# fu5ha/rayn

Hardware: NVIDIA H100
Metric: Msamples/sec (pixels x spp) (higher is better)
Workload: dtype f32

## Files before the change

### rayn_b200/csrc/api.cu

```cuda
#include <cuda_runtime.h>
#include <dlfcn.h>
#include <limits.h>
#include <stdarg.h>
#include <stdio.h>
#include <string.h>

#include <algorithm>
#include <array>
#include <string>
#include <vector>

#include "rt_accum.cuh"
#include "rt_denoise.cuh"
#include "rt_first_hit.cuh"
#include "rt_kernels.cuh"
#include "rt_temporal.cuh"
#ifdef RAYN_LEGACY_KERNELS
#include "rt_legacy.cuh"
#endif

using namespace rt;

static thread_local std::string g_last_error;

// ... 27 lines not shown
  float* d_slabs = nullptr;
  size_t cap_slabs = 0;
};

struct PassBuf {
  void** ptr;
  size_t per_path, per_slot, per_tile, fixed;
};
static const int N_PASS_BUFS = 23;

struct JobPlane {
  float* user;
  int floats;
};

struct RaynContext {
  int device = 0;
  int flags = 0;
  cudaStream_t stream = nullptr;
  std::string err;
  bool has_scene = false;
  DevScene scene;
  int64_t cap_paths = 0;
  size_t pass_cap[N_PASS_BUFS] = {};
  PassBufs pb;
  int* d_tile_ids = nullptr;
  int* d_batch_prefix = nullptr;
  int* d_work_ctr = nullptr;
  int n_sm = 148;
  int occ_ext[2][SDFV_COUNT], occ_shd[SDFV_COUNT], occ_nrm[SDFV_COUNT], occ_nrm_trap[SDFV_COUNT];
  int occ_pre = 8, occ_post = 8, occ_sph = 8;
  int occ_pre_trap = 8, occ_post_trap = 8;
  int sdf_var[RAYN_MAX_HITABLES];
  struct Div3Check { float min_r2, fixed_r2; bool ok; };
  std::vector<Div3Check> div3_cache;
  float *d_s1 = nullptr, *d_s2 = nullptr, *d_scr = nullptr, *d_fis = nullptr;
  size_t cap_s1 = 0, cap_s2 = 0, cap_scr = 0;
  float* d_planes = nullptr;
  size_t cap_planes = 0;
  int* d_pack_ids = nullptr;
  size_t cap_pack_ids = 0;
  unsigned char* d_post = nullptr;
  size_t cap_post = 0;
// ... 47 lines not shown
    if (r_ != 0)                                                                                     \
      return fail(ctx, RAYN_ERR_NCCL, "%s: %s (%s:%d)", #call, g_nccl.GetErrorString ? g_nccl.GetErrorString(r_) : "?", __FILE__, __LINE__); \
  } while (0)

template <class T>
static cudaError_t regrow(T** p, size_t* cap, size_t need) {
  if (need <= *cap && *p) return cudaSuccess;
  if (*p) cudaFree(*p);
  *p = nullptr;
  *cap = 0;
  cudaError_t e = cudaMalloc((void**)p, std::max<size_t>(need, 1) * sizeof(T));
  if (e == cudaSuccess) *cap = need;
  return e;
}

static std::array<PassBuf, N_PASS_BUFS> pass_table(RaynContext* c, int QS, int seg_per_path, int lc_ns, bool trap) {
  PassBufs& p = c->pb;
  const size_t nseg = (QS + SEG_SLOTS - 1) / SEG_SLOTS;
  return {{
      {(void**)&p.o_time, sizeof(float4), 0, 0, 0},
      {(void**)&p.d_t, sizeof(float4), 0, 0, 0},
      {(void**)&p.rad, sizeof(float4), 0, 0, 0},
      {(void**)&p.thr, sizeof(float4), 0, 0, 0},
      {(void**)&p.nrm0, sizeof(float4), 0, 0, 0},
      {(void**)&p.term, sizeof(uint32_t), 0, 0, 0},
      {(void**)&p.q_live, sizeof(int), 0, 0, 0},
      {(void**)&p.q_key, sizeof(int), 0, 0, 0},
      {(void**)&p.q_shade, 0, sizeof(int), 0, 0},
      {(void**)&p.n_live, 0, 0, sizeof(int), 0},
      {(void**)&p.n_slots, 0, 0, sizeof(int), 0},
      {(void**)&p.bin_start, 0, 0, (RAYN_MAX_HITABLES + 1) * sizeof(int), 0},
      {(void**)&c->d_tile_ids, 0, 0, sizeof(int), 0},
      {(void**)&c->d_batch_prefix, 0, 0, sizeof(int), sizeof(int)},
      {(void**)&p.seg_cnt, 0, 0, nseg * RAYN_MAX_HITABLES * sizeof(int), 0},
      {(void**)&p.slot_prefix, 0, 0, (1 + RAYN_MAX_HITABLES) * sizeof(int), (1 + RAYN_MAX_HITABLES) * sizeof(int)},
      {(void**)&p.nrm, sizeof(float4), 0, 0, 0},
      {(void**)&p.vis, sizeof(uint32_t), 0, 0, 0},
      {(void**)&p.seg_a, (size_t)seg_per_path * sizeof(float4), 0, 0, 0},
      {(void**)&p.seg_b, (size_t)seg_per_path * sizeof(float4), 0, 0, 0},
      {(void**)&p.lc_c, (size_t)lc_ns * sizeof(float4), 0, 0, 0},
      {(void**)&p.lc_t, lc_ns > 4 ? 8 * sizeof(float) : 0, 0, 0, 0},
      {(void**)&p.trap_s, trap ? sizeof(float) : 0, 0, 0, 0},
  }};
}

static void free_pass(RaynContext* c) {
  for (const PassBuf& b : pass_table(c, 0, 0, 0, false)) {
    cudaFree(*b.ptr);
    *b.ptr = nullptr;
  }
  unsigned long long* counters = c->pb.counters;
  memset(&c->pb, 0, sizeof c->pb);
  c->pb.counters = counters;
  memset(c->pass_cap, 0, sizeof c->pass_cap);
}

static size_t pass_bytes_per_path(RaynContext* c, int R, int QS, int seg_per_path, int lc_ns, bool trap) {
  size_t bytes = 0;
  for (const PassBuf& b : pass_table(c, QS, seg_per_path, lc_ns, trap))
    bytes += b.per_path + (b.per_slot ? (size_t)(((double)QS / R) * b.per_slot + 1) : 0);
  return bytes;
}

static int32_t ensure_pass(RaynContext* ctx, int n_tiles, int R, int QS, int seg_per_path, int n_sdf, int lc_ns, bool trap) {
  const int64_t need_paths = (int64_t)n_tiles * R, need_q = (int64_t)n_tiles * QS;
  const std::array<PassBuf, N_PASS_BUFS> table = pass_table(ctx, QS, seg_per_path, lc_ns, trap);
  size_t need[N_PASS_BUFS];
  bool fits = true;
  for (int i = 0; i < N_PASS_BUFS; ++i) {
    const PassBuf& b = table[i];
    need[i] = b.per_path * need_paths + b.per_slot * need_q + b.per_tile * n_tiles + b.fixed;
    fits = fits && need[i] <= ctx->pass_cap[i];
  }
  if (fits) return RAYN_OK;
  free_pass(ctx);
  for (int i = 0; i < N_PASS_BUFS; ++i) {
    if (need[i] == 0) continue;
    const cudaError_t e = cudaMalloc(table[i].ptr, need[i]);
    if (e != cudaSuccess) {
      cudaGetLastError();
      free_pass(ctx);
      return fail(ctx, e == cudaErrorMemoryAllocation ? RAYN_ERR_OOM : RAYN_ERR_CUDA, "pass buffers (%lld paths): %s", (long long)need_paths,
                  cudaGetErrorString(e));
    }
    ctx->pass_cap[i] = need[i];
  }
  ctx->pb.prefix_stride = n_tiles + 1;
  ctx->pb.seg_cap = n_sdf > 0 ? need_paths * seg_per_path / n_sdf : 0;
  return RAYN_OK;
}

static void timed_begin(RaynContext* ctx, int kernel) {
  if (!(ctx->flags & RAYN_FLAG_TIMING)) return;
  if (ctx->timed_used == ctx->timed.size()) {
    TimedLaunch t;
    t.kernel = kernel;
    cudaEventCreate(&t.a);
    cudaEventCreate(&t.b);
    ctx->timed.push_back(t);
  }
  ctx->timed[ctx->timed_used].kernel = kernel;
  cudaEventRecord(ctx->timed[ctx->timed_used].a, ctx->stream);
}
// ... 67 lines not shown
  if (cudaGetDeviceCount(&ndev) != cudaSuccess || ndev == 0) {
    cudaGetLastError();
    return fail(nullptr, RAYN_ERR_NO_DEVICE, "no CUDA device: the rayn_b200 render path has no CPU fallback");
  }
  const int dev = cfg ? cfg->device : 0;
  if (dev < 0 || dev >= ndev) return fail(nullptr, RAYN_ERR_INVALID_ARG, "device %d out of range (have %d)", dev, ndev);
#ifndef RAYN_LEGACY_KERNELS
  if (cfg && (cfg->flags & RAYN_FLAG_SIMPLE_MARCH))
    return fail(nullptr, RAYN_ERR_UNSUPPORTED, "RAYN_FLAG_SIMPLE_MARCH needs the test build (librayn_b200_legacy.so, -DRAYN_LEGACY_KERNELS)");
#endif
  CU(cudaSetDevice(dev));
  ctx = new RaynContext();
  ctx->device = dev;
  ctx->flags = cfg ? cfg->flags : 0;
  ctx->cap_paths = (cfg && cfg->max_paths_per_pass > 0) ? cfg->max_paths_per_pass : (int64_t)96 << 20;
  memset(&ctx->pb, 0, sizeof ctx->pb);
  memset(&ctx->stats, 0, sizeof ctx->stats);
  memset(&ctx->scene, 0, sizeof ctx->scene);
  cudaError_t e = cudaStreamCreateWithFlags(&ctx->stream, cudaStreamNonBlocking);
  if (e == cudaSuccess) e = cudaMalloc(&ctx->pb.counters, CNT_TOTAL * sizeof(unsigned long long));
  if (e == cudaSuccess) e = cudaMalloc(&ctx->d_fis, RAYN_FIS_TABLE_SIZE * sizeof(float));
  if (e == cudaSuccess) e = cudaMalloc(&ctx->d_work_ctr, WC_TOTAL * sizeof(int));
  if (e == cudaSuccess) e = cudaMalloc(&ctx->d_kat, sizeof(unsigned long long));
  if (e == cudaSuccess) e = cudaDeviceGetAttribute(&ctx->n_sm, cudaDevAttrMultiProcessorCount, dev);
  if (e == cudaSuccess) e = cudaEventCreate(&ctx->ev0);
  if (e == cudaSuccess) e = cudaEventCreate(&ctx->ev1);
  for (int v = 0; v < SDFV_COUNT && e == cudaSuccess; ++v) {
    DISPATCH_SDFV(v, e = cudaOccupancyMaxActiveBlocksPerMultiprocessor(&ctx->occ_ext[0][v], k_extend_march<V, false>, EXT_T, 0);
                  if (e == cudaSuccess) e = cudaOccupancyMaxActiveBlocksPerMultiprocessor(&ctx->occ_ext[1][v], k_extend_march<V, true>, EXT_T, 0);
                  if (e == cudaSuccess) e = cudaOccupancyMaxActiveBlocksPerMultiprocessor(&ctx->occ_shd[v], k_shadow<V>, SHD_T, 0);
                  if (e == cudaSuccess) e = cudaOccupancyMaxActiveBlocksPerMultiprocessor(&ctx->occ_nrm[v], k_normals<V, false>, SLOT_BLOCK, 0);
                  if (e == cudaSuccess) e = cudaOccupancyMaxActiveBlocksPerMultiprocessor(&ctx->occ_nrm_trap[v], k_normals<V, true>, SLOT_BLOCK, 0));
  }
  if (e == cudaSuccess) e = cudaOccupancyMaxActiveBlocksPerMultiprocessor(&ctx->occ_pre, k_shade_pre<false>, SLOT_BLOCK, 0);
  if (e == cudaSuccess) e = cudaOccupancyMaxActiveBlocksPerMultiprocessor(&ctx->occ_post, k_shade_post<false>, SLOT_BLOCK, 0);
  if (e == cudaSuccess) e = cudaOccupancyMaxActiveBlocksPerMultiprocessor(&ctx->occ_pre_trap, k_shade_pre<true>, SLOT_BLOCK, 0);
  if (e == cudaSuccess) e = cudaOccupancyMaxActiveBlocksPerMultiprocessor(&ctx->occ_post_trap, k_shade_post<true>, SLOT_BLOCK, 0);
  if (e == cudaSuccess) e = cudaOccupancyMaxActiveBlocksPerMultiprocessor(&ctx->occ_sph, k_extend_spheres, EXT_BATCH, 0);
  if (e != cudaSuccess) {
    cudaGetLastError();
    fail(nullptr, RAYN_ERR_CUDA, "context setup: %s", cudaGetErrorString(e));
    if (ctx->stream) cudaStreamDestroy(ctx->stream);
    cudaFree(ctx->pb.counters), cudaFree(ctx->d_fis), cudaFree(ctx->d_work_ctr), cudaFree(ctx->d_kat);
    if (ctx->ev0) cudaEventDestroy(ctx->ev0);
    if (ctx->ev1) cudaEventDestroy(ctx->ev1);
    delete ctx;
    return RAYN_ERR_CUDA;
  }
  *out_ctx = ctx;
  return RAYN_OK;
}

int32_t rayn_b200_comm_destroy(RaynContext* ctx) {
  if (!ctx) return RAYN_ERR_INVALID_ARG;
  RaynComm& c = ctx->comm;
  cudaSetDevice(ctx->device);
  cudaStreamSynchronize(ctx->stream);
  if (c.comm && g_nccl.CommDestroy) g_nccl.CommDestroy(c.comm);
  cudaFree(c.d_table), cudaFree(c.d_slabs);
  c = RaynComm();
  return RAYN_OK;
}

void rayn_b200_destroy(RaynContext* ctx) {
  if (!ctx) return;
  cudaSetDevice(ctx->device);
  cudaStreamSynchronize(ctx->stream);
  rayn_b200_comm_destroy(ctx);
  free_pass(ctx);
  cudaFree(ctx->pb.counters);
  cudaFree(ctx->d_work_ctr);
  cudaFree(ctx->d_kat);
  cudaFree(ctx->d_pack_ids);
  cudaFree(ctx->d_post);
  cudaFree(ctx->d_s1), cudaFree(ctx->d_s2), cudaFree(ctx->d_scr), cudaFree(ctx->d_fis), cudaFree(ctx->d_planes);
  cudaFree(ctx->d_prev);
  for (auto& t : ctx->timed) cudaEventDestroy(t.a), cudaEventDestroy(t.b);
  if (ctx->graph_exec) cudaGraphExecDestroy(ctx->graph_exec);
  cudaEventDestroy(ctx->ev0), cudaEventDestroy(ctx->ev1);
  cudaStreamDestroy(ctx->stream);
  delete ctx;
}

static int32_t validate_scene(RaynContext* ctx, const RaynSceneDesc* s) {
  if (!s) return fail(ctx, RAYN_ERR_INVALID_ARG, "scene is NULL");
  if (s->n_hitables < 1 || s->n_hitables > RAYN_MAX_HITABLES)
    return fail(ctx, RAYN_ERR_INVALID_ARG, "n_hitables %d not in [1,%d]", s->n_hitables, RAYN_MAX_HITABLES);
  if (s->n_materials < 1 || s->n_materials > RAYN_MAX_MATERIALS)
    return fail(ctx, RAYN_ERR_INVALID_ARG, "n_materials %d not in [1,%d]", s->n_materials, RAYN_MAX_MATERIALS);
  if (s->n_lights < 0 || s->n_lights > RAYN_MAX_LIGHTS)
    return fail(ctx, RAYN_ERR_INVALID_ARG, "n_lights %d not in [0,%d]", s->n_lights, RAYN_MAX_LIGHTS);
  if (!s->hitables || !s->materials || (s->n_lights && !s->lights)) return fail(ctx, RAYN_ERR_INVALID_ARG, "NULL scene array");
  for (int i = 0; i < s->n_hitables; ++i) {
    const RaynHitable& h = s->hitables[i];
    if (h.kind < 0 || h.kind > RAYN_HITABLE_MANDELBULB) return fail(ctx, RAYN_ERR_INVALID_ARG, "hitable %d: bad kind %d", i, h.kind);
// ... 123 lines not shown
}

}

struct FramePlan {
  DevFrame fr;
  int R, QS, np, wpc;
  bool simple, traps, fold_all, volume_on;
  int fold_pre, n_fold, ns, seg_per_path, lc_ns;
};

struct Job {
  FramePlan P;
  PassBufs pb;
  int tiles_per_pass;
};

static unsigned resident(const RaynContext* ctx, const Job& J, int occ) {
  const int64_t max_blocks = (int64_t)J.pb.n_tiles * ((J.P.QS + SLOT_BLOCK - 1) / SLOT_BLOCK);
  return (unsigned)std::max<int64_t>(1, std::min<int64_t>((int64_t)ctx->n_sm * occ, max_blocks));
}

static int32_t frame_check(RaynContext* ctx, const RaynFrameDesc* f, bool tiles_given, FramePlan* P) {
  if (f->width <= 0 || f->height <= 0 || f->tile_w <= 0 || f->tile_h <= 0 || f->samples <= 0 || f->max_bounces < 0)
    return fail(ctx, RAYN_ERR_INVALID_ARG, "bad frame geometry");
  if (f->volume_marches != 2)
    return fail(ctx, RAYN_ERR_UNSUPPORTED, "volume_marches = %d: the reference hard-wires samples_1d[3],[4] for vm = 2", f->volume_marches);
  const int spp = 4 * f->samples, vm = f->volume_marches, mb = f->max_bounces;
  const int need1 = 1 + (mb + 1) * (3 + vm), need2 = 2 + (mb + 1) * (12 + 8 * vm) / 2;
  if (f->sets_1d < need1 || f->sets_2d < need2)
// ... 63 lines not shown
  int& fold_pre = P->fold_pre;
  fold_pre = -1;
  if (!motion && !simple) {
    fold_pre = 0;
    while (fold_pre < n_hit && ctx->scene.hit[fold_pre].kind == RAYN_HITABLE_SPHERE) ++fold_pre;
  }
  const bool fold_all = P->fold_all = fold_pre >= 0 && n_sdf == 1 && ctx->scene.hit[ctx->scene.sdf_idx[0]].kind == RAYN_HITABLE_MANDELBOX && !(ctx->flags & RAYN_FLAG_NO_FOLD_ALL);
  P->n_fold = fold_all ? ctx->scene.n_sph : fold_pre;
  const bool volume_on = P->volume_on = ctx->scene.vol.has_scattering != 0 && ctx->scene.n_lights > 0;
  const int ns = P->ns = volume_on ? 4 * (1 + vm) : 4;
  P->seg_per_path = simple ? 0 : ns * n_sdf;
  P->lc_ns = simple ? 0 : ns;
  return RAYN_OK;
}

static int32_t size_pass(RaynContext* ctx, const FramePlan& P, size_t n_tiles, int* out_tiles_per_pass) {
  const int R = P.R, QS = P.QS, n_sdf = ctx->scene.n_sdf, ns = P.ns, seg_per_path = P.seg_per_path, lc_ns = P.lc_ns;
  const bool traps = P.traps;
  const size_t bpp = pass_bytes_per_path(ctx, R, QS, seg_per_path, lc_ns, traps);
  size_t free_b = 0, total_b = 0, pass_bytes = 0;
  CU(cudaMemGetInfo(&free_b, &total_b));
  for (size_t b : ctx->pass_cap) pass_bytes += b;
  const size_t budget = (size_t)((double)(free_b + pass_bytes) * 0.90);
  int64_t max_paths = std::min<int64_t>(ctx->cap_paths, (int64_t)(budget / bpp));
  if (n_sdf > 0) max_paths = std::min<int64_t>(max_paths, ((int64_t)1 << 27) - 1);
  if (n_sdf > 0) max_paths = std::min<int64_t>(max_paths, (int64_t)INT_MAX / std::max(ns, 1));
  int& tiles_per_pass = *out_tiles_per_pass;
  tiles_per_pass = (int)std::max<int64_t>(1, max_paths / R);
  tiles_per_pass = std::min(tiles_per_pass, 65535);
  tiles_per_pass = std::min<int>(tiles_per_pass, (int)std::max<size_t>(n_tiles, 1));
  int32_t rc;
  while ((rc = ensure_pass(ctx, tiles_per_pass, R, QS, seg_per_path, n_sdf, lc_ns, traps)) == RAYN_ERR_OOM && tiles_per_pass > 1)
    tiles_per_pass = (tiles_per_pass + 1) / 2;
  return rc;
}

static int32_t extend_enqueue(RaynContext* ctx, const Job& J, const Thr& thr) {
  cudaStream_t st = ctx->stream;
  const PassBufs& pb = J.pb;
  const int n_hit = ctx->scene.n_hit, fold_pre = J.P.fold_pre;
  const bool fold_all = J.P.fold_all, motion = ctx->scene.sph_moving != 0;
  const unsigned sph_grid = resident(ctx, J, ctx->occ_sph);
  timed_begin(ctx, RAYN_K_MISC);
  k_scan_live<<<1, SCAN_T, 0, st>>>(pb, ctx->d_batch_prefix, ctx->d_work_ctr);
  timed_end(ctx, RAYN_K_MISC);
  int k = fold_pre >= 0 ? fold_pre : 0, first_kernel = fold_pre >= 0 ? 0 : 1, n_march = 0;
  while (k < n_hit || first_kernel) {
    int e = k;
    while (e < n_hit && ctx->scene.hit[e].kind == RAYN_HITABLE_SPHERE) ++e;
    if ((e > k || first_kernel) && !fold_all) {
      timed_begin(ctx, RAYN_K_EXTEND_SPHERES);
      k_extend_spheres<<<sph_grid, EXT_BATCH, 0, st>>>(ctx->scene, pb, k, e, first_kernel, motion ? 1 : 0, ctx->d_batch_prefix, ctx->d_work_ctr + WC_SPHERES + k);
      timed_end(ctx, RAYN_K_EXTEND_SPHERES);
      first_kernel = 0;
    }
    if (e < n_hit) {
      if (n_march++ > 0) CU(cudaMemsetAsync(ctx->d_work_ctr + WC_EXTEND, 0, sizeof(int), st));
      const int v = ctx->sdf_var[e];
      timed_begin(ctx, RAYN_K_EXTEND);
      const int sf = fold_all ? 1 : 0;
      if (thr.is_const)
        DISPATCH_SDFV(v, (k_extend_march<V, true><<<ctx->n_sm * ctx->occ_ext[1][v], EXT_T, 0, st>>>(ctx->scene, pb, thr, e, sf, ctx->d_batch_prefix, ctx->d_work_ctr + WC_EXTEND)))
      else
        DISPATCH_SDFV(v, (k_extend_march<V, false><<<ctx->n_sm * ctx->occ_ext[0][v], EXT_T, 0, st>>>(ctx->scene, pb, thr, e, sf, ctx->d_batch_prefix, ctx->d_work_ctr + WC_EXTEND)))
      timed_end(ctx, RAYN_K_EXTEND);
      ++e;
    }
    k = e;
  }
  return RAYN_OK;
}


static int32_t job_ready(RaynContext* ctx, const char* call) {
  if (!ctx) return fail(nullptr, RAYN_ERR_INVALID_ARG, "ctx is NULL");
  if (ctx->pending) return fail(ctx, RAYN_ERR_INVALID_ARG, "a render is already in flight on this context");
  if (!ctx->has_scene) return fail(ctx, RAYN_ERR_NO_SCENE, "%s before upload_scene", call);
  return RAYN_OK;
}
// ... 19 lines not shown
      my_tiles.push_back(idx);
    }
  } else {
    for (int idx = f->tile_offset; idx < fr.ntx * fr.nty; idx += stride) my_tiles.push_back(idx);
  }
  ctx->job_w = f->width, ctx->job_h = f->height, ctx->job_tw = f->tile_w, ctx->job_th = f->tile_h, ctx->job_spp = fr.spp, ctx->job_nty = fr.nty;
  ctx->job_out.clear();

  memset(&ctx->stats, 0, sizeof ctx->stats);
  ctx->timed_used = 0;
  if (render) ctx->qlog.clear();
  if (f->input_space == RAYN_MEM_DEVICE || out_space == RAYN_MEM_DEVICE) CU(cudaDeviceSynchronize());
  CU(cudaEventRecord(ctx->ev0, ctx->stream));
  if ((rc = upload_tables(ctx, f, &P.fr))) return rc;
  if ((rc = scene_plan(ctx, &P))) return rc;
  if ((rc = size_pass(ctx, P, my_tiles.size(), &J->tiles_per_pass))) return rc;
  PassBufs& pb = J->pb = ctx->pb;
  pb.R = P.R, pb.QS = P.QS, pb.tile_ids = ctx->d_tile_ids;
  pb.lc_ns = P.lc_ns;
  pb.seg_count = ctx->d_work_ctr + WC_SEG_COUNT;
  CU(cudaMemsetAsync(pb.counters, 0, CNT_TOTAL * sizeof(unsigned long long), ctx->stream));
  return RAYN_OK;
}

static int32_t pass_tiles(RaynContext* ctx, Job* J, size_t first) {
  const int nt = J->pb.n_tiles = (int)std::min<size_t>(J->tiles_per_pass, ctx->job_tiles.size() - first);
  CU(cudaMemcpyAsync(ctx->d_tile_ids, ctx->job_tiles.data() + first, nt * sizeof(int), cudaMemcpyHostToDevice, ctx->stream));
  return RAYN_OK;
}

static int32_t job_stage(RaynContext* ctx, const JobPlane* planes, int n, bool zero, float** stage) {
  const size_t npx = (size_t)ctx->job_w * ctx->job_h;
  size_t floats = 0;
  for (int i = 0; i < n; ++i) floats += planes[i].floats;
  CU(regrow(&ctx->d_planes, &ctx->cap_planes, floats * npx));
  if (zero) CU(cudaMemsetAsync(ctx->d_planes, 0, floats * npx * sizeof(float), ctx->stream));
  floats = 0;
  for (int i = 0; i < n; ++i) stage[i] = ctx->d_planes + floats * npx, floats += planes[i].floats;
  ctx->job_out.assign(planes, planes + n);
  return RAYN_OK;
}

static void pass_raygen(RaynContext* ctx, const Job& J) {
  ctx->stats.passes++;
  timed_begin(ctx, RAYN_K_RAYGEN);
  k_raygen<<<dim3((J.P.R + 255) / 256, J.pb.n_tiles), 256, 0, ctx->stream>>>(ctx->scene, J.P.fr, J.pb, J.P.n_fold);
  timed_end(ctx, RAYN_K_RAYGEN);
}

static int32_t render_enqueue(RaynContext* ctx, const RaynFrameDesc* f, const RaynFilmPlanes* out, const std::vector<int>* tiles_override,
                              RaynFilmPlanes* dev_planes_out, const RaynMomentPlanes* moments) {
  int32_t rc = job_ready(ctx, "render_frame");
  if (rc) return rc;
  if (!f || !out) return fail(ctx, RAYN_ERR_INVALID_ARG, "frame/out is NULL");
  Job J;
  if ((rc = job_begin(ctx, f, tiles_override, true, out->space, &J))) return rc;
  const FramePlan& P = J.P;
  const DevFrame& fr = P.fr;
  PassBufs& pb = J.pb;
  const std::vector<int>& my_tiles = ctx->job_tiles;
  const bool mom = moments != nullptr;
  const int mb = fr.max_bounces, np = P.np, wpc = mom ? resolve_warps_per_cta(np, true) : P.wpc, R = P.R, QS = P.QS, n_hit = ctx->scene.n_hit, n_sdf = ctx->scene.n_sdf, n_fold = P.n_fold;
  const int* sdf_idx = ctx->scene.sdf_idx;
  const bool simple = P.simple, motion = ctx->scene.sph_moving != 0, traps = P.traps, volume_on = P.volume_on;
  cudaStream_t st = ctx->stream;

  if (mom && wpc < 1) return fail(ctx, RAYN_ERR_UNSUPPORTED, "render_frame_moments: spp = %d does not fit the film resolve's shared memory", fr.spp);
  const size_t npx = (size_t)f->width * f->height;
  RaynFilmPlanes dp = *out;
  float *dm_color = mom ? moments->color_lum2 : nullptr, *dm_bg = mom ? moments->background_lum2 : nullptr;
  if (out->space == RAYN_MEM_HOST) {
    const JobPlane planes[6] = {{out->color, 3}, {out->alpha, 1}, {out->background, 3}, {out->normal, 3}, {dm_color, 1}, {dm_bg, 1}};
    float* stage[6];
    if ((rc = job_stage(ctx, planes, mom ? 6 : 4, true, stage))) return rc;
    dp = RaynFilmPlanes{stage[0], stage[1], stage[2], stage[3], RAYN_MEM_DEVICE};
    dm_color = dm_color ? stage[4] : nullptr, dm_bg = dm_bg ? stage[5] : nullptr;
  } else {
    const int cov_w = std::min(fr.ntx * f->tile_w, f->width), cov_h = std::min(fr.nty * f->tile_h, f->height);
    if (cov_w < f->width || cov_h < f->height) {
      k_zero_uncovered<<<(unsigned)((npx + 255) / 256), 256, 0, st>>>(f->width, f->height, cov_w, cov_h, dp.color, dp.alpha, dp.background, dp.normal);
      for (float* m : {dm_color, dm_bg})
        if (m) k_zero_uncovered<<<(unsigned)((npx + 255) / 256), 256, 0, st>>>(f->width, f->height, cov_w, cov_h, nullptr, m, nullptr, nullptr);
    }
  }
  dp.space = RAYN_MEM_DEVICE;
  if (dev_planes_out) *dev_planes_out = dp;

  const size_t res_smem = resolve_smem_per_warp(np, mom) * wpc;
  int slot_bits = 5, depth_bits = 1;
  while ((1 << slot_bits) < QS + 1) ++slot_bits;
  while ((1 << depth_bits) < mb + 1) ++depth_bits;
  CU(cudaFuncSetAttribute(mom ? k_resolve<true> : k_resolve<false>, cudaFuncAttributeMaxDynamicSharedMemorySize, (int)res_smem));

  const bool single_pass = my_tiles.size() <= (size_t)J.tiles_per_pass;
  const bool use_graph = single_pass && !my_tiles.empty() && !(ctx->flags & (RAYN_FLAG_TIMING | RAYN_FLAG_NO_GRAPH)) && !ctx->qlog_enabled &&
                         (int64_t)my_tiles.size() * R <= ((int64_t)8 << 20);
  bool capturing = false, replayed = false;
  uint64_t key = 0;
  if (use_graph) {
    PassBufs kpb = pb;
    kpb.n_tiles = (int)my_tiles.size();
    key = fnv1a(1469598103934665603ull, &ctx->scene, sizeof ctx->scene);
    key = fnv1a(key, &fr, sizeof fr);
    key = fnv1a(key, &kpb, sizeof kpb);
    float* planes6[6] = {dp.color, dp.alpha, dp.background, dp.normal, dm_color, dm_bg};
    key = fnv1a(key, planes6, sizeof planes6);
    const int misc[7] = {np, wpc, mb, n_fold, simple ? 1 : 0, motion ? 1 : 0, mom ? 1 : 0};
    key = fnv1a(key, misc, sizeof misc);
    key = fnv1a(key, my_tiles.data(), my_tiles.size() * sizeof(int));
    if (ctx->graph_exec && ctx->graph_key == key) {
      CU(cudaMemcpyAsync(ctx->d_tile_ids, my_tiles.data(), my_tiles.size() * sizeof(int), cudaMemcpyHostToDevice, st));
      CU(cudaGraphLaunch(ctx->graph_exec, st));
      ctx->stats = ctx->graph_stats;
      replayed = true;
    }
  }
  std::vector<int> h_nslots, h_slots;
  for (size_t first = 0; first < my_tiles.size() && !replayed; first += J.tiles_per_pass) {
    if ((rc = pass_tiles(ctx, &J, first))) return rc;
    if (use_graph) {
      CU(cudaStreamBeginCapture(st, cudaStreamCaptureModeThreadLocal));
      capturing = true;
    }
    pass_raygen(ctx, J);
    const int nt = pb.n_tiles;
    const int nseg = (QS + SEG_SLOTS - 1) / SEG_SLOTS;
    for (int depth = 0; depth <= mb; ++depth) {
      const Thr thr = make_thr(ctx->scene.cam, depth);
      if (simple) {
#ifdef RAYN_LEGACY_KERNELS
        timed_begin(ctx, RAYN_K_EXTEND);
        k_extend<<<dim3((R + 127) / 128, nt), 128, 0, st>>>(ctx->scene, pb, thr);
        timed_end(ctx, RAYN_K_EXTEND);
#endif
// ... 14 lines not shown
        for (int t = 0; t < nt; ++t) {
          ctx->qlog.push_back(depth);
          ctx->qlog.push_back(my_tiles[first + t]);
          ctx->qlog.push_back(h_nslots[t]);
          for (int s = 0; s < h_nslots[t]; ++s) ctx->qlog.push_back(h_slots[(size_t)t * QS + s]);
        }
      }
      if (!simple) {
        for (int j = 0; j < n_sdf; ++j) {
          const RaynHitable& h = ctx->scene.hit[sdf_idx[j]];
          const int mk = ctx->scene.mat[h.material].kind;
          if (!(mk == RAYN_MATERIAL_LAMBERTIAN || mk == RAYN_MATERIAL_DIELECTRIC || volume_on)) continue;
          const int v = ctx->sdf_var[sdf_idx[j]];
          timed_begin(ctx, RAYN_K_NORMALS);
          if ((ctx->scene.trap_mask >> h.material) & 1u)
            DISPATCH_SDFV(v, (k_normals<V, true><<<resident(ctx, J, ctx->occ_nrm_trap[v]), SLOT_BLOCK, 0, st>>>(ctx->scene, pb, thr, sdf_idx[j], j, ctx->d_work_ctr + WC_NORMALS + j)))
          else
            DISPATCH_SDFV(v, (k_normals<V, false><<<resident(ctx, J, ctx->occ_nrm[v]), SLOT_BLOCK, 0, st>>>(ctx->scene, pb, thr, sdf_idx[j], j, ctx->d_work_ctr + WC_NORMALS + j)))
          timed_end(ctx, RAYN_K_NORMALS);
        }
        timed_begin(ctx, RAYN_K_SHADE_PRE);
        if (traps)
          k_shade_pre<true><<<resident(ctx, J, ctx->occ_pre_trap), SLOT_BLOCK, 0, st>>>(ctx->scene, fr, pb, depth, thr, ctx->d_work_ctr + WC_PRE);
        else
          k_shade_pre<false><<<resident(ctx, J, ctx->occ_pre), SLOT_BLOCK, 0, st>>>(ctx->scene, fr, pb, depth, thr, ctx->d_work_ctr + WC_PRE);
        timed_end(ctx, RAYN_K_SHADE_PRE);
        if (ctx->scene.n_lights > 0) {
          for (int j = 0; j < n_sdf; ++j) {
            const int v = ctx->sdf_var[sdf_idx[j]];
            timed_begin(ctx, RAYN_K_SHADOW);
            DISPATCH_SDFV(v, (k_shadow<V><<<ctx->n_sm * ctx->occ_shd[v], SHD_T, 0, st>>>(ctx->scene, pb, sdf_idx[j], j, ctx->d_work_ctr + WC_SHADOW + j)));
            timed_end(ctx, RAYN_K_SHADOW);
          }
        }
        timed_begin(ctx, RAYN_K_SHADE_POST);
        if (traps)
          k_shade_post<true><<<resident(ctx, J, ctx->occ_post_trap), SLOT_BLOCK, 0, st>>>(ctx->scene, fr, pb, depth, n_fold, ctx->d_work_ctr + WC_POST);
        else
          k_shade_post<false><<<resident(ctx, J, ctx->occ_post), SLOT_BLOCK, 0, st>>>(ctx->scene, fr, pb, depth, n_fold, ctx->d_work_ctr + WC_POST);
        timed_end(ctx, RAYN_K_SHADE_POST);
      } else {
#ifdef RAYN_LEGACY_KERNELS
        timed_begin(ctx, RAYN_K_SHADE_PRE);
        k_shade<<<dim3((QS + 127) / 128, nt), 128, 0, st>>>(ctx->scene, fr, pb, depth, thr);
        timed_end(ctx, RAYN_K_SHADE_PRE);
#endif
      }
      if (depth < mb) {
        timed_begin(ctx, RAYN_K_COMPACT);
        k_compact_count<<<dim3(nseg, nt), CMP_T, 0, st>>>(pb, nseg);
        k_compact_scatter<<<dim3(nseg, nt), CMP_T, 0, st>>>(pb, nseg);
        timed_end(ctx, RAYN_K_COMPACT, 2);
      }
    }
// ... 49 lines not shown
  return RAYN_OK;
}

static int32_t job_end(RaynContext* ctx, int32_t rc = RAYN_OK) {
  if (!rc) rc = copy_out(ctx);
  const int32_t rc2 = render_finish(ctx);
  return rc ? rc : rc2;
}

static int32_t render_finish(RaynContext* ctx) {
  if (!ctx->pending) return RAYN_OK;
  ctx->pending = false;
  cudaStream_t st = ctx->stream;
  CU(cudaSetDevice(ctx->device));
  CU(cudaEventRecord(ctx->ev1, st));
  CU(cudaMemcpyAsync(ctx->h_counters, ctx->pb.counters, sizeof ctx->h_counters, cudaMemcpyDeviceToHost, st));
  CU(cudaStreamSynchronize(st));
  CU(cudaGetLastError());
  CU(cudaEventElapsedTime(&ctx->stats.total_ms, ctx->ev0, ctx->ev1));
  const unsigned long long* h = ctx->h_counters;
  ctx->stats.extend_rays = (int64_t)h[CNT_EXTEND_RAYS];
  ctx->stats.shade_lanes = (int64_t)h[CNT_SHADE_LANES];
  ctx->stats.shadow_rays = (int64_t)h[CNT_SHADOW_RAYS];
  ctx->stats.sdf_evals_extend = (int64_t)h[CNT_EVALS_EXTEND];
  ctx->stats.sdf_evals_shadow = (int64_t)h[CNT_EVALS_SHADOW];
  ctx->stats.sdf_evals_normals = (int64_t)h[CNT_EVALS_NORMALS];
  ctx->stats.bulb_iters_extend = (int64_t)h[CNT_BULB_ITERS_EXTEND];
  ctx->stats.bulb_iters_shadow = (int64_t)h[CNT_BULB_ITERS_SHADOW];
  ctx->stats.march_trips_extend = (int64_t)h[CNT_TRIPS_EXTEND];
  ctx->stats.march_trips_shadow = (int64_t)h[CNT_TRIPS_SHADOW];
  {
// ... 170 lines not shown
  }
  float *dm = motion ? dev[0] : nullptr, *da = albedo ? dev[1] : nullptr;
  if (prev) {
    if (!ctx->d_prev) CU(cudaMalloc(&ctx->d_prev, sizeof(DevPrev)));
    CU(cudaMemcpyAsync(ctx->d_prev, &dp, sizeof dp, cudaMemcpyHostToDevice, st));
  }
  if (dm) k_motion_clear<<<(unsigned)((npx + 255) / 256), 256, 0, st>>>((long long)npx, dm);
  if (da) CU(cudaMemsetAsync(da, 0, npx * 3 * sizeof(float), st));
  typedef void (*PathsKernel)(DevScene, DevFrame, PassBufs, float, const DevPrev*);
  static const PathsKernel motion_paths[2][2] = {
      {k_first_hit_paths<true, false, false>, k_first_hit_paths<true, true, false>},
      {k_first_hit_paths<true, false, true>, k_first_hit_paths<true, true, true>}};
  const PathsKernel paths = dm ? motion_paths[prev != nullptr][da != nullptr] : k_first_hit_paths<false, true, false>;
  const Thr thr = make_thr(ctx->scene.cam, 0);
  for (size_t first = 0; first < ctx->job_tiles.size(); first += J.tiles_per_pass) {
    if ((rc = pass_tiles(ctx, &J, first))) return rc;
    pass_raygen(ctx, J);
    if ((rc = extend_enqueue(ctx, J, thr))) return rc;
    const dim3 gp((J.P.R + 255) / 256, pb.n_tiles), gr((f->tile_w * f->tile_h + 255) / 256, pb.n_tiles);
    timed_begin(ctx, RAYN_K_NORMALS);
    paths<<<gp, 256, 0, st>>>(ctx->scene, fr, pb, frame_dt, prev ? ctx->d_prev : nullptr);
    timed_end(ctx, RAYN_K_NORMALS);
    timed_begin(ctx, RAYN_K_RESOLVE);
    if (dm) k_motion_resolve<<<gr, 256, 0, st>>>(fr, pb, pb.rad, dm);
    if (da) k_albedo_resolve<<<gr, 256, 0, st>>>(fr, pb, pb.nrm, da);
    timed_end(ctx, RAYN_K_RESOLVE, (dm ? 1 : 0) + (da ? 1 : 0));
    CU(cudaGetLastError());
  }
  ctx->pending = true;
  return job_end(ctx);
}
// ... 795 lines not shown
```

Before: 368.2.

## Double-buffer pass buffers across two streams to overlap consecutive render passes

Splits the per-pass buffers into two sets, each with its own stream, work counters and tile ids. When a frame needs several passes, it halves the memory budget per set and alternates passes between the two streams with fork/join events. Persistent march and shadow grids are halved when paired so both passes can run at once. This targets idle SM time in the tail of each pass and in serial per-bounce launches, at the cost of smaller passes and possible contention between them.

After: 379.7 (median of 6 runs). +3.1%, better.

```diff
diff --git a/rayn_b200/csrc/api.cu b/rayn_b200/csrc/api.cu
--- a/rayn_b200/csrc/api.cu
+++ b/rayn_b200/csrc/api.cu
@@ -65,6 +65,15 @@
   int floats;
 };
 
+struct PassSet {
+  cudaStream_t stream = nullptr;
+  size_t cap[N_PASS_BUFS] = {};
+  PassBufs pb;
+  int* d_tile_ids = nullptr;
+  int* d_batch_prefix = nullptr;
+  int* d_work_ctr = nullptr;
+};
+
 struct RaynContext {
   int device = 0;
   int flags = 0;
@@ -73,11 +82,9 @@
   bool has_scene = false;
   DevScene scene;
   int64_t cap_paths = 0;
-  size_t pass_cap[N_PASS_BUFS] = {};
-  PassBufs pb;
-  int* d_tile_ids = nullptr;
-  int* d_batch_prefix = nullptr;
-  int* d_work_ctr = nullptr;
+  PassSet ps[2];
+  unsigned long long* d_counters = nullptr;
+  cudaEvent_t ev_fork = nullptr, ev_join = nullptr;
   int n_sm = 148;
   int occ_ext[2][SDFV_COUNT], occ_shd[SDFV_COUNT], occ_nrm[SDFV_COUNT], occ_nrm_trap[SDFV_COUNT];
   int occ_pre = 8, occ_post = 8, occ_sph = 8;
@@ -155,7 +162,7 @@
   return e;
 }
 
-static std::array<PassBuf, N_PASS_BUFS> pass_table(RaynContext* c, int QS, int seg_per_path, int lc_ns, bool trap) {
+static std::array<PassBuf, N_PASS_BUFS> pass_table(PassSet* c, int QS, int seg_per_path, int lc_ns, bool trap) {
   PassBufs& p = c->pb;
   const size_t nseg = (QS + SEG_SLOTS - 1) / SEG_SLOTS;
   return {{
@@ -185,49 +192,55 @@
   }};
 }
 
-static void free_pass(RaynContext* c) {
-  for (const PassBuf& b : pass_table(c, 0, 0, 0, false)) {
+static void free_pass(PassSet* s) {
+  for (const PassBuf& b : pass_table(s, 0, 0, 0, false)) {
     cudaFree(*b.ptr);
     *b.ptr = nullptr;
   }
-  unsigned long long* counters = c->pb.counters;
-  memset(&c->pb, 0, sizeof c->pb);
-  c->pb.counters = counters;
-  memset(c->pass_cap, 0, sizeof c->pass_cap);
-}
-
-static size_t pass_bytes_per_path(RaynContext* c, int R, int QS, int seg_per_path, int lc_ns, bool trap) {
+  unsigned long long* counters = s->pb.counters;
+  memset(&s->pb, 0, sizeof s->pb);
+  s->pb.counters = counters;
+  memset(s->cap, 0, sizeof s->cap);
+}
+
+static size_t pass_set_bytes(const PassSet& s) {
   size_t bytes = 0;
-  for (const PassBuf& b : pass_table(c, QS, seg_per_path, lc_ns, trap))
+  for (size_t b : s.cap) bytes += b;
+  return bytes;
+}
+
+static size_t pass_bytes_per_path(PassSet* s, int R, int QS, int seg_per_path, int lc_ns, bool trap) {
+  size_t bytes = 0;
+  for (const PassBuf& b : pass_table(s, QS, seg_per_path, lc_ns, trap))
     bytes += b.per_path + (b.per_slot ? (size_t)(((double)QS / R) * b.per_slot + 1) : 0);
   return bytes;
 }
 
-static int32_t ensure_pass(RaynContext* ctx, int n_tiles, int R, int QS, int seg_per_path, int n_sdf, int lc_ns, bool trap) {
+static int32_t ensure_pass(RaynContext* ctx, PassSet* s, int n_tiles, int R, int QS, int seg_per_path, int n_sdf, int lc_ns, bool trap) {
   const int64_t need_paths = (int64_t)n_tiles * R, need_q = (int64_t)n_tiles * QS;
-  const std::array<PassBuf, N_PASS_BUFS> table = pass_table(ctx, QS, seg_per_path, lc_ns, trap);
+  const std::array<PassBuf, N_PASS_BUFS> table = pass_table(s, QS, seg_per_path, lc_ns, trap);
   size_t need[N_PASS_BUFS];
   bool fits = true;
   for (int i = 0; i < N_PASS_BUFS; ++i) {
     const PassBuf& b = table[i];
     need[i] = b.per_path * need_paths + b.per_slot * need_q + b.per_tile * n_tiles + b.fixed;
-    fits = fits && need[i] <= ctx->pass_cap[i];
+    fits = fits && need[i] <= s->cap[i];
   }
   if (fits) return RAYN_OK;
-  free_pass(ctx);
+  free_pass(s);
   for (int i = 0; i < N_PASS_BUFS; ++i) {
     if (need[i] == 0) continue;
     const cudaError_t e = cudaMalloc(table[i].ptr, need[i]);
     if (e != cudaSuccess) {
       cudaGetLastError();
-      free_pass(ctx);
+      free_pass(s);
       return fail(ctx, e == cudaErrorMemoryAllocation ? RAYN_ERR_OOM : RAYN_ERR_CUDA, "pass buffers (%lld paths): %s", (long long)need_paths,
                   cudaGetErrorString(e));
     }
-    ctx->pass_cap[i] = need[i];
-  }
-  ctx->pb.prefix_stride = n_tiles + 1;
-  ctx->pb.seg_cap = n_sdf > 0 ? need_paths * seg_per_path / n_sdf : 0;
+    s->cap[i] = need[i];
+  }
+  s->pb.prefix_stride = n_tiles + 1;
+  s->pb.seg_cap = n_sdf > 0 ? need_paths * seg_per_path / n_sdf : 0;
   return RAYN_OK;
 }
 
@@ -325,17 +338,24 @@
   ctx->device = dev;
   ctx->flags = cfg ? cfg->flags : 0;
   ctx->cap_paths = (cfg && cfg->max_paths_per_pass > 0) ? cfg->max_paths_per_pass : (int64_t)96 << 20;
-  memset(&ctx->pb, 0, sizeof ctx->pb);
   memset(&ctx->stats, 0, sizeof ctx->stats);
   memset(&ctx->scene, 0, sizeof ctx->scene);
   cudaError_t e = cudaStreamCreateWithFlags(&ctx->stream, cudaStreamNonBlocking);
-  if (e == cudaSuccess) e = cudaMalloc(&ctx->pb.counters, CNT_TOTAL * sizeof(unsigned long long));
+  if (e == cudaSuccess) e = cudaStreamCreateWithFlags(&ctx->ps[1].stream, cudaStreamNonBlocking);
+  ctx->ps[0].stream = ctx->stream;
+  if (e == cudaSuccess) e = cudaMalloc(&ctx->d_counters, CNT_TOTAL * sizeof(unsigned long long));
   if (e == cudaSuccess) e = cudaMalloc(&ctx->d_fis, RAYN_FIS_TABLE_SIZE * sizeof(float));
-  if (e == cudaSuccess) e = cudaMalloc(&ctx->d_work_ctr, WC_TOTAL * sizeof(int));
+  for (PassSet& s : ctx->ps) {
+    memset(&s.pb, 0, sizeof s.pb);
+    s.pb.counters = ctx->d_counters;
+    if (e == cudaSuccess) e = cudaMalloc(&s.d_work_ctr, WC_TOTAL * sizeof(int));
+  }
   if (e == cudaSuccess) e = cudaMalloc(&ctx->d_kat, sizeof(unsigned long long));
   if (e == cudaSuccess) e = cudaDeviceGetAttribute(&ctx->n_sm, cudaDevAttrMultiProcessorCount, dev);
   if (e == cudaSuccess) e = cudaEventCreate(&ctx->ev0);
   if (e == cudaSuccess) e = cudaEventCreate(&ctx->ev1);
+  if (e == cudaSuccess) e = cudaEventCreateWithFlags(&ctx->ev_fork, cudaEventDisableTiming);
+  if (e == cudaSuccess) e = cudaEventCreateWithFlags(&ctx->ev_join, cudaEventDisableTiming);
   for (int v = 0; v < SDFV_COUNT && e == cudaSuccess; ++v) {
     DISPATCH_SDFV(v, e = cudaOccupancyMaxActiveBlocksPerMultiprocessor(&ctx->occ_ext[0][v], k_extend_march<V, false>, EXT_T, 0);
                   if (e == cudaSuccess) e = cudaOccupancyMaxActiveBlocksPerMultiprocessor(&ctx->occ_ext[1][v], k_extend_march<V, true>, EXT_T, 0);
@@ -352,9 +372,10 @@
     cudaGetLastError();
     fail(nullptr, RAYN_ERR_CUDA, "context setup: %s", cudaGetErrorString(e));
     if (ctx->stream) cudaStreamDestroy(ctx->stream);
-    cudaFree(ctx->pb.counters), cudaFree(ctx->d_fis), cudaFree(ctx->d_work_ctr), cudaFree(ctx->d_kat);
-    if (ctx->ev0) cudaEventDestroy(ctx->ev0);
-    if (ctx->ev1) cudaEventDestroy(ctx->ev1);
+    if (ctx->ps[1].stream) cudaStreamDestroy(ctx->ps[1].stream);
+    cudaFree(ctx->d_counters), cudaFree(ctx->d_fis), cudaFree(ctx->ps[0].d_work_ctr), cudaFree(ctx->ps[1].d_work_ctr), cudaFree(ctx->d_kat);
+    for (cudaEvent_t ev : {ctx->ev0, ctx->ev1, ctx->ev_fork, ctx->ev_join})
+      if (ev) cudaEventDestroy(ev);
     delete ctx;
     return RAYN_ERR_CUDA;
   }
@@ -377,10 +398,13 @@
   if (!ctx) return;
   cudaSetDevice(ctx->device);
   cudaStreamSynchronize(ctx->stream);
+  cudaStreamSynchronize(ctx->ps[1].stream);
   rayn_b200_comm_destroy(ctx);
-  free_pass(ctx);
-  cudaFree(ctx->pb.counters);
-  cudaFree(ctx->d_work_ctr);
+  for (PassSet& s : ctx->ps) {
+    free_pass(&s);
+    cudaFree(s.d_work_ctr);
+  }
+  cudaFree(ctx->d_counters);
   cudaFree(ctx->d_kat);
   cudaFree(ctx->d_pack_ids);
   cudaFree(ctx->d_post);
@@ -388,8 +412,8 @@
   cudaFree(ctx->d_prev);
   for (auto& t : ctx->timed) cudaEventDestroy(t.a), cudaEventDestroy(t.b);
   if (ctx->graph_exec) cudaGraphExecDestroy(ctx->graph_exec);
-  cudaEventDestroy(ctx->ev0), cudaEventDestroy(ctx->ev1);
-  cudaStreamDestroy(ctx->stream);
+  cudaEventDestroy(ctx->ev0), cudaEventDestroy(ctx->ev1), cudaEventDestroy(ctx->ev_fork), cudaEventDestroy(ctx->ev_join);
+  cudaStreamDestroy(ctx->stream), cudaStreamDestroy(ctx->ps[1].stream);
   delete ctx;
 }
 
@@ -543,6 +567,10 @@
   FramePlan P;
   PassBufs pb;
   int tiles_per_pass;
+  int n_sets;
+  bool paired;
+  cudaStream_t st;
+  int *batch_prefix, *work_ctr;
 };
 
 static unsigned resident(const RaynContext* ctx, const Job& J, int occ) {
@@ -636,35 +664,67 @@
   return RAYN_OK;
 }
 
-static int32_t size_pass(RaynContext* ctx, const FramePlan& P, size_t n_tiles, int* out_tiles_per_pass) {
+static int32_t size_pass(RaynContext* ctx, const FramePlan& P, size_t n_tiles, bool two_sets, int* out_tiles_per_pass, int* out_sets) {
   const int R = P.R, QS = P.QS, n_sdf = ctx->scene.n_sdf, ns = P.ns, seg_per_path = P.seg_per_path, lc_ns = P.lc_ns;
   const bool traps = P.traps;
-  const size_t bpp = pass_bytes_per_path(ctx, R, QS, seg_per_path, lc_ns, traps);
-  size_t free_b = 0, total_b = 0, pass_bytes = 0;
+  const size_t bpp = pass_bytes_per_path(&ctx->ps[0], R, QS, seg_per_path, lc_ns, traps);
+  size_t free_b = 0, total_b = 0;
   CU(cudaMemGetInfo(&free_b, &total_b));
-  for (size_t b : ctx->pass_cap) pass_bytes += b;
-  const size_t budget = (size_t)((double)(free_b + pass_bytes) * 0.90);
-  int64_t max_paths = std::min<int64_t>(ctx->cap_paths, (int64_t)(budget / bpp));
-  if (n_sdf > 0) max_paths = std::min<int64_t>(max_paths, ((int64_t)1 << 27) - 1);
-  if (n_sdf > 0) max_paths = std::min<int64_t>(max_paths, (int64_t)INT_MAX / std::max(ns, 1));
+  const size_t budget = (size_t)((double)(free_b + pass_set_bytes(ctx->ps[0]) + pass_set_bytes(ctx->ps[1])) * 0.90);
+  auto tiles_for = [&](size_t bytes) {
+    int64_t max_paths = std::min<int64_t>(ctx->cap_paths, (int64_t)(bytes / bpp));
+    if (n_sdf > 0) max_paths = std::min<int64_t>(max_paths, ((int64_t)1 << 27) - 1);
+    if (n_sdf > 0) max_paths = std::min<int64_t>(max_paths, (int64_t)INT_MAX / std::max(ns, 1));
+    return std::min<int64_t>(max_paths / R, 65535);
+  };
+  int64_t tiles = tiles_for(budget);
+  const bool several = tiles < (int64_t)n_tiles, halves = several && tiles_for(budget / 2) >= 1;
+  if (halves) tiles = tiles_for(budget / 2);
   int& tiles_per_pass = *out_tiles_per_pass;
-  tiles_per_pass = (int)std::max<int64_t>(1, max_paths / R);
-  tiles_per_pass = std::min(tiles_per_pass, 65535);
+  tiles_per_pass = (int)std::max<int64_t>(1, tiles);
   tiles_per_pass = std::min<int>(tiles_per_pass, (int)std::max<size_t>(n_tiles, 1));
   int32_t rc;
-  while ((rc = ensure_pass(ctx, tiles_per_pass, R, QS, seg_per_path, n_sdf, lc_ns, traps)) == RAYN_ERR_OOM && tiles_per_pass > 1)
+  while ((rc = ensure_pass(ctx, &ctx->ps[0], tiles_per_pass, R, QS, seg_per_path, n_sdf, lc_ns, traps)) == RAYN_ERR_OOM) {
+    if (pass_set_bytes(ctx->ps[1])) {
+      free_pass(&ctx->ps[1]);
+      continue;
+    }
+    if (tiles_per_pass == 1) break;
     tiles_per_pass = (tiles_per_pass + 1) / 2;
+  }
+  *out_sets = 1;
+  if (rc || !two_sets || !halves || (size_t)tiles_per_pass >= n_tiles) return rc;
+  rc = ensure_pass(ctx, &ctx->ps[1], tiles_per_pass, R, QS, seg_per_path, n_sdf, lc_ns, traps);
+  if (rc == RAYN_ERR_OOM) return RAYN_OK;
+  if (rc == RAYN_OK) {
+    *out_sets = 2;
+    const size_t passes = (n_tiles + tiles_per_pass - 1) / tiles_per_pass;
+    tiles_per_pass = (int)((n_tiles + passes - 1) / passes);
+  }
   return rc;
 }
 
+static void pass_set_use(RaynContext* ctx, Job* J, int set) {
+  PassSet& s = ctx->ps[set];
+  PassBufs& pb = J->pb = s.pb;
+  pb.R = J->P.R, pb.QS = J->P.QS, pb.tile_ids = s.d_tile_ids;
+  pb.lc_ns = J->P.lc_ns;
+  pb.seg_count = s.d_work_ctr + WC_SEG_COUNT;
+  J->st = s.stream, J->batch_prefix = s.d_batch_prefix, J->work_ctr = s.d_work_ctr;
+}
+
+static unsigned march_grid(const RaynContext* ctx, const Job& J, int occ) {
+  return (unsigned)ctx->n_sm * (J.paired ? (occ + 1) / 2 : occ);
+}
+
 static int32_t extend_enqueue(RaynContext* ctx, const Job& J, const Thr& thr) {
-  cudaStream_t st = ctx->stream;
+  cudaStream_t st = J.st;
   const PassBufs& pb = J.pb;
   const int n_hit = ctx->scene.n_hit, fold_pre = J.P.fold_pre;
   const bool fold_all = J.P.fold_all, motion = ctx->scene.sph_moving != 0;
   const unsigned sph_grid = resident(ctx, J, ctx->occ_sph);
   timed_begin(ctx, RAYN_K_MISC);
-  k_scan_live<<<1, SCAN_T, 0, st>>>(pb, ctx->d_batch_prefix, ctx->d_work_ctr);
+  k_scan_live<<<1, SCAN_T, 0, st>>>(pb, J.batch_prefix, J.work_ctr);
   timed_end(ctx, RAYN_K_MISC);
   int k = fold_pre >= 0 ? fold_pre : 0, first_kernel = fold_pre >= 0 ? 0 : 1, n_march = 0;
   while (k < n_hit || first_kernel) {
@@ -672,19 +732,19 @@
     while (e < n_hit && ctx->scene.hit[e].kind == RAYN_HITABLE_SPHERE) ++e;
     if ((e > k || first_kernel) && !fold_all) {
       timed_begin(ctx, RAYN_K_EXTEND_SPHERES);
-      k_extend_spheres<<<sph_grid, EXT_BATCH, 0, st>>>(ctx->scene, pb, k, e, first_kernel, motion ? 1 : 0, ctx->d_batch_prefix, ctx->d_work_ctr + WC_SPHERES + k);
+      k_extend_spheres<<<sph_grid, EXT_BATCH, 0, st>>>(ctx->scene, pb, k, e, first_kernel, motion ? 1 : 0, J.batch_prefix, J.work_ctr + WC_SPHERES + k);
       timed_end(ctx, RAYN_K_EXTEND_SPHERES);
       first_kernel = 0;
     }
     if (e < n_hit) {
-      if (n_march++ > 0) CU(cudaMemsetAsync(ctx->d_work_ctr + WC_EXTEND, 0, sizeof(int), st));
+      if (n_march++ > 0) CU(cudaMemsetAsync(J.work_ctr + WC_EXTEND, 0, sizeof(int), st));
       const int v = ctx->sdf_var[e];
       timed_begin(ctx, RAYN_K_EXTEND);
       const int sf = fold_all ? 1 : 0;
       if (thr.is_const)
-        DISPATCH_SDFV(v, (k_extend_march<V, true><<<ctx->n_sm * ctx->occ_ext[1][v], EXT_T, 0, st>>>(ctx->scene, pb, thr, e, sf, ctx->d_batch_prefix, ctx->d_work_ctr + WC_EXTEND)))
+        DISPATCH_SDFV(v, (k_extend_march<V, true><<<march_grid(ctx, J, ctx->occ_ext[1][v]), EXT_T, 0, st>>>(ctx->scene, pb, thr, e, sf, J.batch_prefix, J.work_ctr + WC_EXTEND)))
       else
-        DISPATCH_SDFV(v, (k_extend_march<V, false><<<ctx->n_sm * ctx->occ_ext[0][v], EXT_T, 0, st>>>(ctx->scene, pb, thr, e, sf, ctx->d_batch_prefix, ctx->d_work_ctr + WC_EXTEND)))
+        DISPATCH_SDFV(v, (k_extend_march<V, false><<<march_grid(ctx, J, ctx->occ_ext[0][v]), EXT_T, 0, st>>>(ctx->scene, pb, thr, e, sf, J.batch_prefix, J.work_ctr + WC_EXTEND)))
       timed_end(ctx, RAYN_K_EXTEND);
       ++e;
     }
@@ -734,18 +794,18 @@
   CU(cudaEventRecord(ctx->ev0, ctx->stream));
   if ((rc = upload_tables(ctx, f, &P.fr))) return rc;
   if ((rc = scene_plan(ctx, &P))) return rc;
-  if ((rc = size_pass(ctx, P, my_tiles.size(), &J->tiles_per_pass))) return rc;
-  PassBufs& pb = J->pb = ctx->pb;
-  pb.R = P.R, pb.QS = P.QS, pb.tile_ids = ctx->d_tile_ids;
-  pb.lc_ns = P.lc_ns;
-  pb.seg_count = ctx->d_work_ctr + WC_SEG_COUNT;
-  CU(cudaMemsetAsync(pb.counters, 0, CNT_TOTAL * sizeof(unsigned long long), ctx->stream));
-  return RAYN_OK;
-}
-
-static int32_t pass_tiles(RaynContext* ctx, Job* J, size_t first) {
+  const bool two_sets = render && !(ctx->flags & RAYN_FLAG_TIMING) && !ctx->qlog_enabled;
+  if ((rc = size_pass(ctx, P, my_tiles.size(), two_sets, &J->tiles_per_pass, &J->n_sets))) return rc;
+  pass_set_use(ctx, J, 0);
+  J->paired = false;
+  CU(cudaMemsetAsync(ctx->d_counters, 0, CNT_TOTAL * sizeof(unsigned long long), ctx->stream));
+  return RAYN_OK;
+}
+
+static int32_t pass_tiles(RaynContext* ctx, Job* J, size_t first, int set) {
+  pass_set_use(ctx, J, set);
   const int nt = J->pb.n_tiles = (int)std::min<size_t>(J->tiles_per_pass, ctx->job_tiles.size() - first);
-  CU(cudaMemcpyAsync(ctx->d_tile_ids, ctx->job_tiles.data() + first, nt * sizeof(int), cudaMemcpyHostToDevice, ctx->stream));
+  CU(cudaMemcpyAsync(ctx->ps[set].d_tile_ids, ctx->job_tiles.data() + first, nt * sizeof(int), cudaMemcpyHostToDevice, J->st));
   return RAYN_OK;
 }
 
@@ -764,7 +824,7 @@
 static void pass_raygen(RaynContext* ctx, const Job& J) {
   ctx->stats.passes++;
   timed_begin(ctx, RAYN_K_RAYGEN);
-  k_raygen<<<dim3((J.P.R + 255) / 256, J.pb.n_tiles), 256, 0, ctx->stream>>>(ctx->scene, J.P.fr, J.pb, J.P.n_fold);
+  k_raygen<<<dim3((J.P.R + 255) / 256, J.pb.n_tiles), 256, 0, J.st>>>(ctx->scene, J.P.fr, J.pb, J.P.n_fold);
   timed_end(ctx, RAYN_K_RAYGEN);
 }
 
@@ -783,7 +843,6 @@
   const int mb = fr.max_bounces, np = P.np, wpc = mom ? resolve_warps_per_cta(np, true) : P.wpc, R = P.R, QS = P.QS, n_hit = ctx->scene.n_hit, n_sdf = ctx->scene.n_sdf, n_fold = P.n_fold;
   const int* sdf_idx = ctx->scene.sdf_idx;
   const bool simple = P.simple, motion = ctx->scene.sph_moving != 0, traps = P.traps, volume_on = P.volume_on;
-  cudaStream_t st = ctx->stream;
 
   if (mom && wpc < 1) return fail(ctx, RAYN_ERR_UNSUPPORTED, "render_frame_moments: spp = %d does not fit the film resolve's shared memory", fr.spp);
   const size_t npx = (size_t)f->width * f->height;
@@ -798,9 +857,9 @@
   } else {
     const int cov_w = std::min(fr.ntx * f->tile_w, f->width), cov_h = std::min(fr.nty * f->tile_h, f->height);
     if (cov_w < f->width || cov_h < f->height) {
-      k_zero_uncovered<<<(unsigned)((npx + 255) / 256), 256, 0, st>>>(f->width, f->height, cov_w, cov_h, dp.color, dp.alpha, dp.background, dp.normal);
+      k_zero_uncovered<<<(unsigned)((npx + 255) / 256), 256, 0, ctx->stream>>>(f->width, f->height, cov_w, cov_h, dp.color, dp.alpha, dp.background, dp.normal);
       for (float* m : {dm_color, dm_bg})
-        if (m) k_zero_uncovered<<<(unsigned)((npx + 255) / 256), 256, 0, st>>>(f->width, f->height, cov_w, cov_h, nullptr, m, nullptr, nullptr);
+        if (m) k_zero_uncovered<<<(unsigned)((npx + 255) / 256), 256, 0, ctx->stream>>>(f->width, f->height, cov_w, cov_h, nullptr, m, nullptr, nullptr);
     }
   }
   dp.space = RAYN_MEM_DEVICE;
@@ -829,15 +888,30 @@
     key = fnv1a(key, misc, sizeof misc);
     key = fnv1a(key, my_tiles.data(), my_tiles.size() * sizeof(int));
     if (ctx->graph_exec && ctx->graph_key == key) {
-      CU(cudaMemcpyAsync(ctx->d_tile_ids, my_tiles.data(), my_tiles.size() * sizeof(int), cudaMemcpyHostToDevice, st));
-      CU(cudaGraphLaunch(ctx->graph_exec, st));
+      CU(cudaMemcpyAsync(ctx->ps[0].d_tile_ids, my_tiles.data(), my_tiles.size() * sizeof(int), cudaMemcpyHostToDevice, ctx->stream));
+      CU(cudaGraphLaunch(ctx->graph_exec, ctx->stream));
       ctx->stats = ctx->graph_stats;
       replayed = true;
     }
   }
+  struct Join {
+    RaynContext* ctx;
+    bool on;
+    ~Join() {
+      if (on && cudaEventRecord(ctx->ev_join, ctx->ps[1].stream) == cudaSuccess) cudaStreamWaitEvent(ctx->stream, ctx->ev_join, 0);
+    }
+  } join{ctx, false};
+  if (J.n_sets > 1 && !replayed) {
+    CU(cudaEventRecord(ctx->ev_fork, ctx->stream));
+    CU(cudaStreamWaitEvent(ctx->ps[1].stream, ctx->ev_fork, 0));
+    join.on = true;
+  }
   std::vector<int> h_nslots, h_slots;
-  for (size_t first = 0; first < my_tiles.size() && !replayed; first += J.tiles_per_pass) {
-    if ((rc = pass_tiles(ctx, &J, first))) return rc;
+  const size_t n_passes = (my_tiles.size() + J.tiles_per_pass - 1) / J.tiles_per_pass;
+  for (size_t first = 0, k = 0; first < my_tiles.size() && !replayed; first += J.tiles_per_pass, ++k) {
+    if ((rc = pass_tiles(ctx, &J, first, (int)(k % J.n_sets)))) return rc;
+    J.paired = J.n_sets > 1 && !(n_passes % 2 == 1 && k == n_passes - 1);
+    const cudaStream_t st = J.st;
     if (use_graph) {
       CU(cudaStreamBeginCapture(st, cudaStreamCaptureModeThreadLocal));
       capturing = true;
@@ -882,30 +956,30 @@
           const int v = ctx->sdf_var[sdf_idx[j]];
           timed_begin(ctx, RAYN_K_NORMALS);
           if ((ctx->scene.trap_mask >> h.material) & 1u)
-            DISPATCH_SDFV(v, (k_normals<V, true><<<resident(ctx, J, ctx->occ_nrm_trap[v]), SLOT_BLOCK, 0, st>>>(ctx->scene, pb, thr, sdf_idx[j], j, ctx->d_work_ctr + WC_NORMALS + j)))
+            DISPATCH_SDFV(v, (k_normals<V, true><<<resident(ctx, J, ctx->occ_nrm_trap[v]), SLOT_BLOCK, 0, st>>>(ctx->scene, pb, thr, sdf_idx[j], j, J.work_ctr + WC_NORMALS + j)))
           else
-            DISPATCH_SDFV(v, (k_normals<V, false><<<resident(ctx, J, ctx->occ_nrm[v]), SLOT_BLOCK, 0, st>>>(ctx->scene, pb, thr, sdf_idx[j], j, ctx->d_work_ctr + WC_NORMALS + j)))
+            DISPATCH_SDFV(v, (k_normals<V, false><<<resident(ctx, J, ctx->occ_nrm[v]), SLOT_BLOCK, 0, st>>>(ctx->scene, pb, thr, sdf_idx[j], j, J.work_ctr + WC_NORMALS + j)))
           timed_end(ctx, RAYN_K_NORMALS);
         }
         timed_begin(ctx, RAYN_K_SHADE_PRE);
         if (traps)
-          k_shade_pre<true><<<resident(ctx, J, ctx->occ_pre_trap), SLOT_BLOCK, 0, st>>>(ctx->scene, fr, pb, depth, thr, ctx->d_work_ctr + WC_PRE);
+          k_shade_pre<true><<<resident(ctx, J, ctx->occ_pre_trap), SLOT_BLOCK, 0, st>>>(ctx->scene, fr, pb, depth, thr, J.work_ctr + WC_PRE);
         else
-          k_shade_pre<false><<<resident(ctx, J, ctx->occ_pre), SLOT_BLOCK, 0, st>>>(ctx->scene, fr, pb, depth, thr, ctx->d_work_ctr + WC_PRE);
+          k_shade_pre<false><<<resident(ctx, J, ctx->occ_pre), SLOT_BLOCK, 0, st>>>(ctx->scene, fr, pb, depth, thr, J.work_ctr + WC_PRE);
         timed_end(ctx, RAYN_K_SHADE_PRE);
         if (ctx->scene.n_lights > 0) {
           for (int j = 0; j < n_sdf; ++j) {
             const int v = ctx->sdf_var[sdf_idx[j]];
             timed_begin(ctx, RAYN_K_SHADOW);
-            DISPATCH_SDFV(v, (k_shadow<V><<<ctx->n_sm * ctx->occ_shd[v], SHD_T, 0, st>>>(ctx->scene, pb, sdf_idx[j], j, ctx->d_work_ctr + WC_SHADOW + j)));
+            DISPATCH_SDFV(v, (k_shadow<V><<<march_grid(ctx, J, ctx->occ_shd[v]), SHD_T, 0, st>>>(ctx->scene, pb, sdf_idx[j], j, J.work_ctr + WC_SHADOW + j)));
             timed_end(ctx, RAYN_K_SHADOW);
           }
         }
         timed_begin(ctx, RAYN_K_SHADE_POST);
         if (traps)
-          k_shade_post<true><<<resident(ctx, J, ctx->occ_post_trap), SLOT_BLOCK, 0, st>>>(ctx->scene, fr, pb, depth, n_fold, ctx->d_work_ctr + WC_POST);
+          k_shade_post<true><<<resident(ctx, J, ctx->occ_post_trap), SLOT_BLOCK, 0, st>>>(ctx->scene, fr, pb, depth, n_fold, J.work_ctr + WC_POST);
         else
-          k_shade_post<false><<<resident(ctx, J, ctx->occ_post), SLOT_BLOCK, 0, st>>>(ctx->scene, fr, pb, depth, n_fold, ctx->d_work_ctr + WC_POST);
+          k_shade_post<false><<<resident(ctx, J, ctx->occ_post), SLOT_BLOCK, 0, st>>>(ctx->scene, fr, pb, depth, n_fold, J.work_ctr + WC_POST);
         timed_end(ctx, RAYN_K_SHADE_POST);
       } else {
 #ifdef RAYN_LEGACY_KERNELS
@@ -985,7 +1059,7 @@
   cudaStream_t st = ctx->stream;
   CU(cudaSetDevice(ctx->device));
   CU(cudaEventRecord(ctx->ev1, st));
-  CU(cudaMemcpyAsync(ctx->h_counters, ctx->pb.counters, sizeof ctx->h_counters, cudaMemcpyDeviceToHost, st));
+  CU(cudaMemcpyAsync(ctx->h_counters, ctx->d_counters, sizeof ctx->h_counters, cudaMemcpyDeviceToHost, st));
   CU(cudaStreamSynchronize(st));
   CU(cudaGetLastError());
   CU(cudaEventElapsedTime(&ctx->stats.total_ms, ctx->ev0, ctx->ev1));
@@ -1186,7 +1260,7 @@
   const PathsKernel paths = dm ? motion_paths[prev != nullptr][da != nullptr] : k_first_hit_paths<false, true, false>;
   const Thr thr = make_thr(ctx->scene.cam, 0);
   for (size_t first = 0; first < ctx->job_tiles.size(); first += J.tiles_per_pass) {
-    if ((rc = pass_tiles(ctx, &J, first))) return rc;
+    if ((rc = pass_tiles(ctx, &J, first, 0))) return rc;
     pass_raygen(ctx, J);
     if ((rc = extend_enqueue(ctx, J, thr))) return rc;
     const dim3 gp((J.P.R + 255) / 256, pb.n_tiles), gr((f->tile_w * f->tile_h + 255) / 256, pb.n_tiles);
```
